# Luh1124/face-vae

Hardware: AMD Instinct MI355X
Metric: training images/sec (256x256 face-VAE step) (higher is better)
Workload: dtype bf16; 1 GPU; FaceVAE step 256x256 (AFE trunk + reparam + Generator trunk, MSE+KL, Adam); global_batch=32, per_gpu_batch=32, resolution=256, parallelism=dp1

## Files before the change

### face-vae_amd/csrc/conv.hip

```cpp
#include "conv_plan.h"

namespace {

__global__ void weight_prep_c7n_kernel(const float* __restrict__ wp, const float* sigma, bf16* wn, int cout) {
  const float inv = sigma ? 1.f / sigma[0] : 1.f;
  for (int e = blockIdx.x * blockDim.x + threadIdx.x; e < 32 * 448; e += gridDim.x * blockDim.x) {
    const int nn = e / 448, k = e - nn * 448;
    const int co = nn / 7, s = nn - co * 7, r = k >> 6, ci = k & 63;
    const float v = co < cout ? wp[((co * 64 + ci) * 7 + r) * 7 + s] * inv : 0.f;
    wn[e] = (bf16)v;
  }
}

template <typename T>
__device__ __forceinline__ void weight_prep_body(const float* __restrict__ wp, const float* sigma, T* wk, int rows,
                                                 int Kpad, int cout, int cin_valid, int lgCin, int KS, int K,
                                                 int transposed, int bid, int nblk, int smaj = 0) {
  const int total = rows * Kpad;
  const float inv = sigma ? 1.f / sigma[0] : 1.f;
  for (int e = bid * (int)blockDim.x + threadIdx.x; e < total; e += nblk * (int)blockDim.x) {
    int row, k;
    bool kin;
    int tap, c;
    if (smaj == 2) {
// ... 716 lines not shown
  const int dtype = descs[0].dtype;
  for (int i = 0; i < n; ++i) {
    const fv_conv_desc* d = &descs[i];
    int st = check_desc(d);
    if (st) return st;
    FV_REQUIRE(d->dtype == dtype, "weight_prep_multi: one dtype per call");
    FV_REQUIRE(fv_conv_weight_prep_batchable(d), "weight_prep_multi: conv %d needs a special layout", i);
    FV_REQUIRE(w_params[i] && wks[i], "weight_prep_multi: null pointer (conv %d)", i);
    const int ks = d->ksize;
    WPrepMJob j0{w_params[i], sigmas[i], wks[i], wrows(d->cout), kpad_lay(smaj_wk(d), kpad_of(ks, d->cin)),
                 fv_ilog2(d->cin),
                 ks * ks * d->cin, 0, 0, d->cout, d->cin_valid, ks, 0, smaj_wk(d)};
    j0.nb = (int)std::min<long>(fv_cdiv((long)j0.rows * j0.Kpad, 256), 256);
    nb_total = std::max(nb_total, j0.nb);
    m.j[m.n++] = j0;
    if (wts[i]) {
      const int cin_t = pad_pow2_8(d->cout);
      WPrepMJob j1{w_params[i], sigmas[i], wts[i], wrows(d->cin), kpad_lay(smaj_wt(d), kpad_of(ks, cin_t)),
                   fv_ilog2(cin_t),
                   ks * ks * cin_t, 1, 0, d->cout, d->cin_valid, ks, 0, smaj_wt(d)};
      j1.nb = (int)std::min<long>(fv_cdiv((long)j1.rows * j1.Kpad, 256), 256);
      nb_total = std::max(nb_total, j1.nb);
      m.j[m.n++] = j1;
    }
  }
  hipStream_t s = (hipStream_t)stream;
  if (dtype == FV_BF16)
    hipLaunchKernelGGL(weight_prep_multi_kernel<bf16>, dim3(nb_total, m.n), dim3(256), 0, s, m);
  else
    hipLaunchKernelGGL(weight_prep_multi_kernel<float>, dim3(nb_total, m.n), dim3(256), 0, s, m);
  return fv_check_launch("weight_prep_multi");
}

static int sr_geometry(const fv_conv_desc* d, int* bp) {
  if (d->dtype != FV_BF16 || use_c7n(d) || halo_tr(d) || use_subpix(d) || use_c64(d)) return 0;
  const int bn = halo3_bn(d);
  const long P = (long)d->n * d->h * d->w;
  if (!bn || d->cout % bn || P % 256) return 0;
  const int nw = bn == 64 ? 4 : 8;
  if (bp) *bp = 256 / nw;
  return (int)(P / 256 * nw);
}

extern "C++" {
static int cu_count() {
  static int n = 0;
  if (!n) {
    int dev = 0;
    if (hipGetDevice(&dev) != hipSuccess || hipDeviceGetAttribute(&n, hipDeviceAttributeMultiprocessorCount, dev) != hipSuccess ||
        n <= 0)
      n = 256;
  }
  return n;
}
static bool halo_epi_ok(const ConvArgs& a, int bn, int tr) {
  return a.lgtw == 6 && !a.sub && !a.nchw && a.W % 64 == 0 && a.H % tr == 0 && a.P == a.N * a.H * a.W &&
         a.ntn * bn == a.Cout && a.ldy >= a.Cout;
}
static int launch_h3(int bn, int mode, int ntiles, hipStream_t s, const ConvArgs& a, unsigned xb) {
  const int sch = res_sched(2) >= 2 ? 2 : 0;
  const char* e = getenv("FV_PERS_GRID");
  const int cap = (e && atoi(e) > 0) ? atoi(e) : cu_count();
  const bool pers = bn < 256 && ntiles > cap;
  if (!launch_halo3_fwd3(a, bn, mode, sch, pers, pers ? cap : ntiles, xb, ntiles, s)) return FV_OK;
  fv_set_error("halo 3x3 conv variant unsupported (co tile %d, mode %d)", bn, mode);
  return FV_E_BADARG;
}
static int launch_h2(int bn, int nblk, hipStream_t s, const ConvArgs& a, unsigned xb) {
  if (!launch_halo3_fwd2(a, bn, nblk, xb, s)) return FV_OK;
  fv_set_error("halo 3x3 conv variant unsupported (co tile %d)", bn);
  return FV_E_BADARG;
}
}

static bool use_c1s(const fv_conv_desc* d) {
  const char* e = getenv("FV_C1S");
  if (e && e[0] == '0') return false;
  if (!use_v2(d) || d->ksize != 1 || d->upsample || d->pro_act) return false;
  if ((d->cin != 256 && d->cin != 512) || d->cout % 256 || d->ldy != d->cout) return false;
  const long P = (long)d->n * d->h * d->w;
  return P % (32768 / d->cin) == 0 && P * d->cout * 2 < (1L << 31);
}

static int conv_run(const fv_conv_desc* d, const void* x, const void* wk, const float* bias,
                    const float* psc, const float* psh, const void* res, void* y, float* stats,
                    hipStream_t s, const fv_store_reduce* sr = nullptr) {
  ConvArgs a{};
  if (sr && sr->mode) {
    FV_REQUIRE(sr_geometry(d, nullptr) > 0, "store-pass records not available for this conv (query fv_conv2d_sr_records)");
    FV_REQUIRE(sr->records, "store-pass records: null buffer");
    FV_REQUIRE(sr->mode == 1 || (sr->mode == 2 && sr->bn_input && sr->mean && sr->invstd && sr->gamma && sr->beta && !res),
               "store-pass records: bad mode / BN arguments");
    FV_REQUIRE(!stats, "store-pass records and accumulator statistics in one call are not supported");
    a.spm = sr->mode;
    a.sprec = sr->records;
    a.bnm = sr->mean; a.bni = sr->invstd; a.bng = sr->gamma; a.bnb = sr->beta; a.bns = sr->slope;
    if (sr->mode == 2) res = sr->bn_input;
  }
  const FwdTile t = fwd_tile(d->cout);
  a.x = x; a.w = wk; a.bias = bias; a.psc = psc; a.psh = psh; a.slope = d->pro_slope;
  a.res = res; a.y = y; a.stats = stats;
  a.nrec = stats ? fv_conv2d_stats_blocks(d) : 0;
  a.N = d->n; a.H = d->h; a.W = d->w;
  a.Hin = d->upsample ? d->h / 2 : d->h;
  a.Win = d->upsample ? d->w / 2 : d->w;
  a.P = d->n * d->h * d->w;
  a.Cin = d->cin; a.lgCin = fv_ilog2(d->cin);
  a.Cout = d->cout; a.ldy = d->ldy;
  a.K = d->ksize * d->ksize * d->cin; a.Kpad = kpad_of(d->ksize, d->cin); a.nks = a.Kpad / BK;
  a.sigmoid = d->epi_sigmoid; a.nchw = d->out_nchw_f32;
  a.ntn = fv_cdiv(d->cout, t.bn);
  int st;
  const long wk_have = (long)fv_conv_wk_elems(d);
  auto wext = [&](long rows, long kk, const char* what) {
    if (rows * kk > wk_have) {
      fv_set_error("conv %s: weight DMA extent %ld x %ld > weight image %ld elements", what, rows, kk, wk_have);
      return FV_E_BADARG;
    }
    return FV_OK;
  };
  if (use_c7n(d)) {
    FV_REQUIRE(!res, "out_conv kernel: no residual");
    const unsigned xb = (unsigned)((long)d->n * d->h * d->w * 64 * 2);
    const int band = c7n_band(d);
    const int nblk = d->n * (d->h / band) * (d->w / 64);
    launch_c7n(a, nblk, xb, band, s);
    return fv_check_launch("conv2d_fwd_c7n2");
  }
  const bool c64 = use_c64(d);
  if (c64 && !res && !a.spm) {
    if ((st = wext(d->cout, kpad_of(3, 64), "c64"))) return st;
    const int nb = c64_bands(d);
    const int nblk = d->n * (d->w / 64) * (d->cout / 64) * nb;
    const unsigned xb = (unsigned)((long)d->n * d->h * d->w * 64 * 2);
    launch_c64(a, nblk, xb, nb, s);
    return fv_check_launch("conv2d_fwd_c64");
  }
  if (use_c74(d)) {
    FV_REQUIRE(!res, "packed 7x7 conv: no residual");
    const int ntiles = d->n * (d->h / C74_TR) * (d->w / 64);
    const unsigned xb = (unsigned)((long)d->n * d->h * d->w * d->cin * 2);
    FV_REQUIRE(!a.stats || a.nrec == c74_grid(d), "packed 7x7 conv: %d BN records for %d blocks", a.nrec, c74_grid(d));
    launch_c74(a, c74_grid(d), xb, ntiles, s);
    return fv_check_launch("conv2d_fwd_c74");
  }
  if (const int tr = halo_tr(d)) {
    if ((st = wext(plan_tile(d).bn, kpad_of(7, d->cin), "halo7"))) return st;
    a.lgtw = 6;
    const int nblk = d->n * (d->h / tr) * (d->w / 64);
    const unsigned xb = (unsigned)((long)d->n * d->h * d->w * d->cin * 2);
    if (launch_halo7(a, d->cin, nblk, xb, s)) {
      fv_set_error("7x7 halo conv variant unsupported (cin=%d)", d->cin);
      return FV_E_BADARG;
    }
    return fv_check_launch("conv2d_fwd_halo");
  }
  if (use_upband(d)) {
    FV_REQUIRE(!res && !a.spm, "sub-pixel band conv: no residual / store-pass records");
    a.Ho = d->h; a.Wo = d->w;
    a.Kpad = kpad_of(2, d->cin);
    a.wphase = wrows(d->cout) * a.Kpad;
    if ((st = wext(4L * wrows(d->cout), a.Kpad, "upband"))) return st;
    const int hl = d->h / 2, wl = d->w / 2;
    const long base = (long)d->n * (wl / 32) * (d->cout / 64);
    int nb = 1;
    while (base * nb < 256 && hl % (nb * 16) == 0) nb *= 2;
    const int nblk = (int)(base * nb);
    const unsigned xb = (unsigned)((long)d->n * hl * wl * 128 * 2);
    launch_upband(a, nblk, xb, nb, s);
    return fv_check_launch("conv2d_fwd_upband");
  }
  if (use_subpix_halo(d)) {
// ... 97 lines not shown
  return fv_check_launch("conv2d_fwd");
}

int fv_conv2d_fwd(const fv_conv_desc* d, const void* x, const void* wk, const float* bias,
                  const float* pro_scale, const float* pro_shift, const void* res, void* y,
                  float* stats, void* stream) {
  int st = check_desc(d);
  if (st) return st;
  FV_REQUIRE(x && wk && y, "null pointer");
  FV_REQUIRE(!d->pro_act || (pro_scale && pro_shift), "prologue needs scale/shift");
  FV_REQUIRE(d->out_nchw_f32 || d->ldy >= d->cout, "ldy < cout");
  FV_REQUIRE(!res || d->ldy % 4 == 0, "residual needs ldy % 4 == 0");
  FV_REQUIRE(d->out_nchw_f32 || d->cout % 4 == 0 || d->ldy >= d->cout, "bad ldy");
  return conv_run(d, x, wk, bias, pro_scale, pro_shift, res, y, stats, (hipStream_t)stream);
}

static fv_conv_desc dgrad_desc(const fv_conv_desc* d) {
  fv_conv_desc t{};
  t.dtype = d->dtype;
  t.n = d->n; t.h = d->h; t.w = d->w;
  t.cin = pad_pow2_8(d->cout);
  t.cin_valid = d->cout;
  t.cout = d->cin;
  t.ldy = d->cin;
  t.ksize = d->ksize;
  return t;
}

int fv_conv2d_sr_records(const fv_conv_desc* d, int dgrad, int* record_pixels) {
  if (check_desc(d) != FV_OK) return 0;
  if (dgrad) {
    if (d->upsample) return 0;
    const fv_conv_desc t = dgrad_desc(d);
    return sr_geometry(&t, record_pixels);
  }
  return sr_geometry(d, record_pixels);
}

int fv_conv2d_fwd_sr(const fv_conv_desc* d, const void* x, const void* wk, const float* bias, const void* res, void* y,
                     const fv_store_reduce* sr, void* stream) {
  int st = check_desc(d);
  if (st) return st;
  FV_REQUIRE(x && wk && y && sr && sr->mode == 1, "fwd_sr: null pointer or mode != 1");
  FV_REQUIRE(!d->pro_act && !d->out_nchw_f32 && d->ldy == d->cout, "fwd_sr: plain NHWC output only");
  return conv_run(d, x, wk, bias, nullptr, nullptr, res, y, nullptr, (hipStream_t)stream, sr);
}

int fv_conv2d_bwd_data_sr(const fv_conv_desc* d, const void* dy, int ldy_dy, const void* wt, void* dx,
                          const fv_store_reduce* sr, void* stream) {
  int st = check_desc(d);
  if (st) return st;
  FV_REQUIRE(dy && wt && dx && sr && sr->mode == 2 && !d->upsample, "bwd_data_sr: bad argument");
  const fv_conv_desc t = dgrad_desc(d);
  FV_REQUIRE(ldy_dy == t.cin, "bwd_data: dy channel stride must be %d (got %d)", t.cin, ldy_dy);
  return conv_run(&t, dy, wt, nullptr, nullptr, nullptr, nullptr, dx, nullptr, (hipStream_t)stream, sr);
}

int fv_conv2d_bwd_data(const fv_conv_desc* d, const void* dy, int ldy_dy, const void* wt, void* dx,
                       void* stream) {
  int st = check_desc(d);
  if (st) return st;
  const fv_conv_desc t = dgrad_desc(d);
  FV_REQUIRE(ldy_dy == t.cin, "bwd_data: dy channel stride must be %d (got %d)", t.cin, ldy_dy);
  if (const int bn = dgrad_halo_bn(d)) {
    FV_REQUIRE(dy && wt && dx, "null pointer");
    ConvArgs a{};
    a.x = dy; a.w = wt; a.y = dx;
// ... 1450 lines not shown
```

### face-vae_amd/csrc/conv_shapes.hip

```cpp
#include "conv_plan.h"

namespace {

template <int KS, int CIN, int RN, int TR, bool WLDS, bool KSPLIT>
__global__ void __launch_bounds__(512, 4)
conv_halo_fwd(ConvArgs a, unsigned x_bytes) {
  constexpr int PAD = KS / 2, TW = 64;
  constexpr int MT = TR * 4;
  constexpr int RM = KSPLIT ? MT : MT / 8;
  constexpr int HR = TR + KS - 1, HW = TW + KS - 1;
  constexpr int CPP = CIN / 8;
  constexpr int HCH = HR * HW * CPP;
  constexpr int HQ = (HCH + 63) / 64;
  constexpr int KPAD = ((KS * KS * CIN + 31) / 32) * 32;
  constexpr int NKS = KPAD / 32;
  constexpr int KPW = (NKS + 7) / 8;
  constexpr int WROW = KPAD / 8 + 1;
  constexpr int WCH = RN * 16 * WROW;
  constexpr int WQ = WLDS ? (WCH + 63) / 64 : 0;
  constexpr int HB = HQ * 1024, WB = WQ * 1024;
  constexpr int SCR = 4096;
  static_assert(!KSPLIT || (RN == 1 && !WLDS && 8 * MT * 1024 <= HB), "k-split layout");
  __shared__ __attribute__((aligned(1024))) char smem[HB + WB + SCR];
  char* halo = smem;
// ... 85 lines not shown
#pragma unroll 2
    for (int ks = ks0; ks < ks1; ++ks) {
      const int kc = ks * 4 + g;
      bf16x8 bfr[RN];
#pragma unroll
      for (int nn = 0; nn < RN; ++nn) {
        if constexpr (WLDS) bfr[nn] = *reinterpret_cast<const bf16x8*>(wlds + ((nn * 16 + li) * WROW + kc) * 16);
        else bfr[nn] = *reinterpret_cast<const bf16x8*>(wk + (long)(nn * 16 + li) * a.Kpad + kc * 8);
      }
      kstep(ks, bfr);
    }
  }
  const int p0 = (n * a.H + h0) * a.W + w0;
  if constexpr (KSPLIT) {
    __syncthreads();
    f32x4* red = reinterpret_cast<f32x4*>(halo);
#pragma unroll
    for (int m = 0; m < RM; ++m) red[(wave * RM + m) * 64 + lane] = acc[0][m];
    __syncthreads();
    f32x4 t[1][1];
    t[0][0] = f32x4{0.f, 0.f, 0.f, 0.f};
#pragma unroll
    for (int w = 0; w < 8; ++w) t[0][0] += red[(w * RM + wave) * 64 + lane];
    conv_epilogue<bf16, 1, 8, 1, 1>(a, t, smem + HB + WB, 0, p0, tile, 0, wave, lane, tid);
  } else {
    conv_epilogue<bf16, 1, 8, RN, RM>(a, acc, smem + HB + WB, 0, p0, tile, 0, wave, lane, tid);
  }
}

constexpr int C74_HW = 71, C74_HR = C74_TR + 6;
constexpr int C74_WCOL = C74_K / 8;
constexpr int C74_WQ = 64 * C74_WCOL / 64;
constexpr int C74_HQ = (C74_HR * C74_HW + 63) / 64;
__global__ void __launch_bounds__(512, 2)
conv7c4_fwd(ConvArgs a, unsigned x_bytes, int ntiles) {
  constexpr int WB = C74_WQ * 1024, HB = C74_HQ * 1024, NHB = 3;
  __shared__ __attribute__((aligned(1024))) char smem[WB + NHB * HB];
  const int tid = threadIdx.x, lane = tid & 63;
  const int wave = __builtin_amdgcn_readfirstlane(tid >> 6);
  const int li = lane & 15, g = lane >> 4;
  const int tiles_w = a.W >> 6, tiles_h = a.H / C74_TR;
  const unsigned sbase = __builtin_amdgcn_readfirstlane((unsigned)(size_t)(lds_ptr_t)smem);
  const __amdgpu_buffer_rsrc_t xr = __builtin_amdgcn_make_buffer_rsrc(const_cast<void*>(a.x), 0, (int)x_bytes, 0x00020000);
  const __amdgpu_buffer_rsrc_t wr = __builtin_amdgcn_make_buffer_rsrc(const_cast<void*>(a.w), 0, 0x7fffffff, 0x00020000);

  auto issue_halo = [&](int tile, int buf) {
    const int n = tile / (tiles_h * tiles_w), rem = tile - n * tiles_h * tiles_w;
    const int h0 = (rem / tiles_w) * C74_TR, w0 = (rem % tiles_w) * 64;
    for (int q = wave; q < C74_HQ; q += 8) {
      const int L = q * 64 + lane;
      const int hr = L / C74_HW, hc = L - (L / C74_HW) * C74_HW;
      const int hh = h0 + hr - 3, ww = w0 + hc - 3;
      const bool ok = L < C74_HR * C74_HW && hh >= 0 && hh < a.H && ww >= 0 && ww < a.W;
      dma16s(xr, sbase + WB + buf * HB + q * 1024, ok ? (unsigned)((((n * a.H + hh) * a.W + ww) * 8) * 2) : 0x80000000u, 0u);
    }
  };
  for (int q = wave; q < C74_WQ; q += 8) {
    const int L = q * 64 + lane;
    const int li = L & 15, t = L >> 4, col = t % C74_WCOL, row = (t / C74_WCOL) * 16 + li;
    dma16s(wr, sbase + q * 1024, (unsigned)((row * C74_K + col * 8) * 2), 0u);
  }
  int tile = blockIdx.x;
  if (tile < ntiles) issue_halo(tile, 0);
  if (tile + (int)gridDim.x < ntiles) issue_halo(tile + gridDim.x, 1);
  asm volatile("s_waitcnt vmcnt(0)" ::: "memory");
  __syncthreads();

  float bv[4][4];
#pragma unroll
  for (int nn = 0; nn < 4; ++nn)
#pragma unroll
    for (int i = 0; i < 4; ++i) bv[nn][i] = a.bias ? a.bias[nn * 16 + g * 4 + i] : 0.f;
  int hbase[2];
#pragma unroll
  for (int m = 0; m < 2; ++m) {
    const int loc = wave * 32 + m * 16 + li;
    hbase[m] = (loc >> 6) * C74_HW + (loc & 63);
  }
  float bs[4][4], bq[4][4];
#pragma unroll
  for (int nn = 0; nn < 4; ++nn)
#pragma unroll
    for (int i = 0; i < 4; ++i) bs[nn][i] = bq[nn][i] = 0.f;
  int buf = 0;
  for (; tile < ntiles; tile += gridDim.x) {
    const int ahead = tile + 2 * gridDim.x;
    if (ahead < ntiles) issue_halo(ahead, buf == 0 ? 2 : buf - 1);
    f32x4 acc[4][2];
#pragma unroll
    for (int nn = 0; nn < 4; ++nn)
#pragma unroll
      for (int m = 0; m < 2; ++m) acc[nn][m] = f32x4{0.f, 0.f, 0.f, 0.f};
    const char* hs = smem + WB + buf * HB;
#pragma unroll
    for (int r = 0; r < 7; ++r) {
      bf16x8 bfr[4], afr[2];
#pragma unroll
      for (int nn = 0; nn < 4; ++nn)
        bfr[nn] = *reinterpret_cast<const bf16x8*>(smem + ((nn * C74_WCOL + r * 4 + g) * 16 + li) * 16);
#pragma unroll
      for (int m = 0; m < 2; ++m) {
        const char* p = hs + (hbase[m] + r * C74_HW + 2 * g) * 16;
        const uint2 lo = *reinterpret_cast<const uint2*>(p), hi = *reinterpret_cast<const uint2*>(p + 16);
        afr[m] = __builtin_bit_cast(bf16x8, make_uint4(lo.x, lo.y, hi.x, hi.y));
      }
#pragma unroll
      for (int nn = 0; nn < 4; ++nn)
#pragma unroll
        for (int m = 0; m < 2; ++m) acc[nn][m] = __builtin_amdgcn_mfma_f32_16x16x32_bf16(bfr[nn], afr[m], acc[nn][m], 0, 0, 0);
    }
    const int n = tile / (tiles_h * tiles_w), rem = tile - n * tiles_h * tiles_w;
    const int p0 = (n * a.H + (rem / tiles_w) * C74_TR) * a.W + (rem % tiles_w) * 64;
#pragma unroll
    for (int nn = 0; nn < 4; ++nn)
#pragma unroll
      for (int m = 0; m < 2; ++m)
#pragma unroll
        for (int i = 0; i < 4; ++i) acc[nn][m][i] += bv[nn][i];
    if (a.stats) {
#pragma unroll
      for (int nn = 0; nn < 4; ++nn)
#pragma unroll
        for (int i = 0; i < 4; ++i) {
          const float v0 = acc[nn][0][i], v1 = acc[nn][1][i];
          bs[nn][i] += v0 + v1;
          bq[nn][i] += v0 * v0 + v1 * v1;
        }
    }
    auto pk = [](float lo, float hi) {
      const bf16 t[2] = {(bf16)lo, (bf16)hi};
      return *reinterpret_cast<const unsigned*>(t);
    };
#pragma unroll
    for (int m = 0; m < 2; ++m) {
      const int loc = wave * 32 + m * 16 + li;
      bf16* yp = reinterpret_cast<bf16*>(a.y) + (long)(p0 + (loc >> 6) * a.W + (loc & 63)) * a.ldy;
#pragma unroll
      for (int q = 0; q < 2; ++q) {
        const f32x4 va = acc[2 * q][m], vb = acc[2 * q + 1][m];
        const auto s0 = __builtin_amdgcn_permlane16_swap(pk(va[0], va[1]), pk(vb[0], vb[1]), false, false);
        const auto s1 = __builtin_amdgcn_permlane16_swap(pk(va[2], va[3]), pk(vb[2], vb[3]), false, false);
        *reinterpret_cast<uint4*>(yp + (2 * q + (g & 1)) * 16 + (g >> 1) * 8) = make_uint4(s0[0], s1[0], s0[1], s1[1]);
      }
    }
    {
      const int dpieces = ahead < ntiles ? (wave + 8 < C74_HQ ? 2 : 1) : 0;
      wait_vm_dyn(8 + dpieces);
    }
    wait_lgkm0();
    __builtin_amdgcn_s_barrier();
    asm volatile("" ::: "memory");
    buf = buf == 2 ? 0 : buf + 1;
  }
  if (a.stats) {
    float* sw = reinterpret_cast<float*>(smem + WB);
#pragma unroll
    for (int nn = 0; nn < 4; ++nn)
#pragma unroll
      for (int i = 0; i < 4; ++i) {
        const float sv = row16_sum(bs[nn][i]), qv = row16_sum(bq[nn][i]);
        if (li == 0) {
          sw[wave * 128 + nn * 16 + g * 4 + i] = sv;
          sw[wave * 128 + 64 + nn * 16 + g * 4 + i] = qv;
        }
      }
    __syncthreads();
    if (tid < 128 && (int)blockIdx.x < a.nrec) {
      float v = 0.f;
#pragma unroll
      for (int w = 0; w < 8; ++w) v += sw[w * 128 + tid];
      a.stats[(long)blockIdx.x * 128 + tid] = v;
    }
  }
}

constexpr int C64_PXB = 160, C64_ROWB = 11 * 1024, C64_NR = 10;
__global__ void __launch_bounds__(512, 1)
conv3c64_fwd(ConvArgs a, unsigned x_bytes, int nbands) {
  __shared__ __attribute__((aligned(1024))) char smem[C64_NR * C64_ROWB];
  __shared__ __attribute__((aligned(16))) float sbias[64];
  __shared__ __attribute__((aligned(16))) float sacc[8 * 16 * 64];
  const int tid = threadIdx.x, lane = tid & 63;
  const int wave = __builtin_amdgcn_readfirstlane(tid >> 6);
  const int cg = wave & 1, rw = wave >> 1;
  const int lr = lane & 15, lh = lane >> 4;
// ... 504 lines not shown
    const int h0 = hb + 4 * j;
    for (int o = tid; o < nout; o += 512) {
      const int co = o / (C7_TR * 64), rr = (o / 64) % C7_TR, w = o % 64;
      float v = co == 0 ? bias4[0] : co == 1 ? bias4[1] : co == 2 ? bias4[2] : bias4[3];
#pragma unroll
      for (int s7 = 0; s7 < 7; ++s7) v += Dl[(rr * 70 + w + s7) * C7B_DLD + co * 7 + s7];
      if (a.stats) {
        const float sv = wave_sum(v), qv = wave_sum(v * v);
        const int rec = ((n * a.H + h0 + rr) * a.W + w0) >> 6;
        if (lane == 0 && rec < a.nrec) {
          a.stats[(long)(rec * 2) * a.Cout + co] = sv;
          a.stats[(long)(rec * 2 + 1) * a.Cout + co] = qv;
        }
      }
      if (a.sigmoid) v = 1.f / (1.f + expf(-v));
      const int pix = (h0 + rr) * a.W + w0 + w;
      if (a.nchw) reinterpret_cast<float*>(a.y)[((long)(n * a.Cout + co)) * HWo + pix] = v;
      else reinterpret_cast<bf16*>(a.y)[((long)n * HWo + pix) * a.ldy + co] = (bf16)v;
    }
  }
}


}

int launch_halo7(const ConvArgs& a, int cin, int nblk, unsigned xb, hipStream_t s) {
  if (cin == 8) hipLaunchKernelGGL((conv_halo_fwd<7, 8, 4, 4, true, false>), dim3(nblk), dim3(512), 0, s, a, xb);
  else if (cin == 64) hipLaunchKernelGGL((conv_halo_fwd<7, 64, 1, 2, false, true>), dim3(nblk), dim3(512), 0, s, a, xb);
  else return FV_E_UNSUPPORTED;
  return FV_OK;
}

void launch_c74(const ConvArgs& a, int grid, unsigned xb, int ntiles, hipStream_t s) {
  hipLaunchKernelGGL(conv7c4_fwd, dim3(grid), dim3(512), 0, s, a, xb, ntiles);
}

void launch_c64(const ConvArgs& a, int nblk, unsigned xb, int nbands, hipStream_t s) {
  hipLaunchKernelGGL(conv3c64_fwd, dim3(nblk), dim3(512), 0, s, a, xb, nbands);
}

void launch_upband(const ConvArgs& a, int nblk, unsigned xb, int nbands, hipStream_t s) {
  hipLaunchKernelGGL(conv3up_band_fwd, dim3(nblk), dim3(512), 0, s, a, xb, nbands);
}

int launch_c1s(const ConvArgs& a, int k, int bpx, int grid, unsigned xb, hipStream_t s) {
  if (k == 256 && bpx == 128) hipLaunchKernelGGL((conv1x1_stream<256, 128>), dim3(grid), dim3(512), 0, s, a, xb);
  else if (k == 256 && bpx == 64) hipLaunchKernelGGL((conv1x1_stream<256, 64>), dim3(grid), dim3(512), 0, s, a, xb);
  else if (k == 512 && bpx == 64) hipLaunchKernelGGL((conv1x1_stream<512, 64>), dim3(grid), dim3(512), 0, s, a, xb);
  else if (k == 512 && bpx == 32) hipLaunchKernelGGL((conv1x1_stream<512, 32>), dim3(grid), dim3(512), 0, s, a, xb);
  else return FV_E_UNSUPPORTED;
  return FV_OK;
}

void launch_c7n(const ConvArgs& a, int nblk, unsigned xb, int band, hipStream_t s) {
  hipLaunchKernelGGL(conv7_n3_fwd2, dim3(nblk), dim3(512), 0, s, a, xb, band);
}
```

### face-vae_amd/ops.py

```python
from __future__ import annotations

import ctypes
import os
import weakref
from typing import Optional

import torch

from . import _lib as L
from ._lib import call, ptr, query, stream

CL = torch.channels_last
F32 = torch.float32
F64 = torch.float64
FP8 = torch.float8_e4m3fn
_FP8_HANDOFF = True


def storage(mode: torch.dtype) -> torch.dtype:
    return torch.bfloat16 if mode == FP8 else mode


def fp8_site(conv, which: str, device):
    sites = conv.__dict__.setdefault("_fv_fp8_sites", {})
    st = sites.get(which)
    if st is None or st[0].device != device:
        st = [torch.zeros(query("fv_fp8_site_bytes") // 4, dtype=torch.int32, device=device), False, []]
        sites[which] = st
    return st


FP8_GLOBAL = None


def _dq_snapshot(site):
    if site is None or len(site) < 3:
        return
    for ref in site[2]:
        cs = ref()
        q = getattr(cs, "x8", None) if cs is not None else None
        if q is not None and q[1].data_ptr() == site[0].data_ptr() + 18 * 4:
            cs.x8 = (q[0], q[1].clone())
    site[2].clear()


_DQ_VIEW = os.environ.get("FV_DQ_VIEW", "1") == "1"


def _hold_x8(cs, x8, xdq, site):
# ... 308 lines not shown
    if stats:
        nb, _ = stats_geometry(cs)
        part = _empty(nb * 2 * d.cout, F32, x.device)
    psc, psh = (pro if pro is not None else (None, None))
    if cs.fp8:
        site = fp8_site(cs.conv, "x", x.device)
        x8, xdq = x8 if x8 is not None else quantize_fp8_site(x, site)
        _hold_x8(cs, x8, xdq, site)
        _timed("fwd", d, lambda: call("fv_conv2d_fwd_fp8_site", ctypes.byref(d), ptr(x8), ptr(site[0]), ptr(cs.wk),
                                      ptr(cs.wdq), ptr(bias), ptr(res), ptr(y), ptr(part), stream()))
        if CHECK is not None:
            CHECK("fwd", cs, x=x, bias=bias, pro=pro, res=res, y=y, q8=(x8, xdq))
        return part
    _timed("fwd", d, lambda: call("fv_conv2d_fwd", ctypes.byref(d), ptr(x), ptr(cs.wk), ptr(bias), ptr(psc),
                                  ptr(psh), ptr(res), ptr(y), ptr(part), stream()))
    if CHECK is not None:
        CHECK("fwd", cs, x=x, bias=bias, pro=pro, res=res, y=y)
    return part


def sr_records(d, dgrad):
    bp = ctypes.c_int(0)
    nrec = query("fv_conv2d_sr_records", ctypes.byref(d), int(dgrad), ctypes.byref(bp))
    return (nrec, bp.value) if nrec > 0 else None


class BNRecords:
    __slots__ = ("part", "nb", "bp", "dx")

    def __init__(self, part, nb, bp, dx):
        self.part, self.nb, self.bp, self.dx = part, nb, bp, dx


def _dgrad_bnred(cs, dy, dx, bnred):
    d = cs.d
    if bnred is None or cs.fp8 or d.upsample or d.dtype != L.FV_BF16:
        return None
    geo = sr_records(d, True)
    if geo is None:
        return None
    bn, r, ybn, slope = bnred
    if r.count == 0 and r.stats is None:
        return None
    nb, bp = geo
    part = _empty(nb * 2 * d.cin, F32, dy.device)
    sr = L.StoreReduce(2, ptr(part), ptr(ybn), ptr(r.mean), ptr(r.invstd), ptr(bn.weight), ptr(bn.bias),
                       float(slope))
    _timed("dgrad", d, lambda: call("fv_conv2d_bwd_data_sr", ctypes.byref(d), ptr(dy), d.cout, ptr(cs.wt), ptr(dx),
                                    ctypes.byref(sr), stream()))
    return BNRecords(part, nb, bp, dx)


def _wgrad(cs: ConvState, x, dy, ldd, pro, need_db):
    d = cs.d
    dev = dy.device
    slab = _empty(query("fv_conv2d_wgrad_slab_elems", ctypes.byref(d)), F32, dev)
    bslab = _empty(query("fv_conv2d_wgrad_bias_slab_elems", ctypes.byref(d)), F32, dev) if need_db else None
    psc, psh = (pro if pro is not None else (None, None))
    _timed("wgrad", d, lambda: call("fv_conv2d_bwd_weight", ctypes.byref(d), ptr(x), ptr(psc), ptr(psh), ptr(dy),
                                    ldd, ptr(slab), ptr(bslab), stream()))
    return _wgrad_finish(cs, x, dy, ldd, pro, need_db, slab, bslab)


def _wgrad_fp8(cs: ConvState, x, dy, ldd, need_db, dy8):
    d = cs.d
    dev = dy.device
    x8, xdq = cs.x8
    dy8_, dydq = dy8
    slab = _empty(query("fv_conv2d_wgrad_slab_elems", ctypes.byref(d)), F32, dev)
    bslab = _empty(query("fv_conv2d_wgrad_bias_slab_elems", ctypes.byref(d)), F32, dev) if need_db else None
    _timed("wgrad", d, lambda: call("fv_conv2d_bwd_weight_fp8", ctypes.byref(d), ptr(x8), ptr(xdq), ptr(dy8_), ptr(dydq),
                                    ptr(slab), ptr(bslab), stream()))
    cs.x8 = None
    return _wgrad_finish(cs, x, dy, ldd, None, need_db, slab, bslab, q8=(x8, xdq, dy8_, dydq))


def _wgrad_finish(cs: ConvState, x, dy, ldd, pro, need_db, slab, bslab, q8=None):
    d = cs.d
    dev = dy.device
    dw = torch.empty_like(cs.w)
    db = torch.empty(d.cout, dtype=F32, device=dev) if need_db else None
# ... 61 lines not shown
        site = fp8_site(cs.conv, "dy", dy.device)
        dy8 = dy8 if dy8 is not None else quantize_fp8_site(dy, site)
        dw, db = _wgrad_fp8(cs, x, dy, ldd, need_db, dy8)
    else:
        if x.numel() == 0 or (dy.numel() == 0 and dy8 is None):
            raise RuntimeError("conv backward: the bf16 operand of this fp8 conv was never materialised "
                               "(FV_Q8_ONLY) and its e4m3 copy was released by an earlier backward; "
                               "backward through an fp8 ResBlock runs once (no retain_graph)")
        dw, db = _wgrad(cs, x, dy, ldd, pro, need_db)
    dx, recs = _dgrad(cs, dy, ldd, need_dx, bnred, dy8)
    return (dx, dw, db, recs) if want_recs else (dx, dw, db)


def _dgrad(cs: ConvState, dy, ldd, need_dx, bnred, dy8=None):
    d = cs.d
    dev = dy.device
    if not need_dx:
        return None, None
    if cs.fp8:
        site = fp8_site(cs.conv, "dy", dy.device)
        dy8, dydq = dy8 if dy8 is not None else quantize_fp8_site(dy, site)
        dx = torch.empty((d.n, d.cin, d.h, d.w), dtype=dy.dtype, device=dev, memory_format=CL)
        _timed("dgrad", d, lambda: call("fv_conv2d_bwd_data_fp8_site", ctypes.byref(d), ptr(dy8), ptr(site[0]),
                                        ptr(cs.wt), ptr(cs.wdq), ptr(dx), stream()))
        if CHECK is not None:
            CHECK("dgrad", cs, dy=dy, ldd=ldd, dx=dx, q8=(dy8, dydq))
        return dx, None
    if d.upsample and query("fv_conv2d_dgrad_lowres", ctypes.byref(d)):
        dx = torch.empty((d.n, d.cin, d.h // 2, d.w // 2), dtype=dy.dtype, device=dev, memory_format=CL)
        _timed("dgrad", d, lambda: call("fv_conv2d_bwd_data", ctypes.byref(d), ptr(dy), ldd, ptr(cs.wt), ptr(dx),
                                        stream()))
    else:
        dx = torch.empty((d.n, d.cin, d.h, d.w), dtype=dy.dtype, device=dev, memory_format=CL)
        recs = _dgrad_bnred(cs, dy, dx, bnred) if ldd == d.cout else None
        if recs is not None:
            if CHECK is not None:
                CHECK("dgrad", cs, dy=dy, ldd=ldd, dx=dx)
            return dx, recs
        _timed("dgrad", d, lambda: call("fv_conv2d_bwd_data", ctypes.byref(d), ptr(dy), ldd, ptr(cs.wt), ptr(dx),
                                        stream()))
        if d.upsample:
            src = torch.empty((d.n, d.cin, d.h // 2, d.w // 2), dtype=dy.dtype, device=dev, memory_format=CL)
            call("fv_upsample2x_bwd", L.dtype_code(dy.dtype), ptr(dx), d.n, d.h // 2, d.w // 2, d.cin, ptr(src),
                 stream())
            dx = src
    if CHECK is not None:
        CHECK("dgrad", cs, dy=dy, ldd=ldd, dx=dx)
    return dx, None



class BNResult:
    __slots__ = ("mean", "invstd", "scale", "shift", "count", "stats")


def _bn_result(C, dev, count, stats=None):
    r = BNResult()
    r.mean = torch.empty(C, dtype=F32, device=dev)
    r.invstd = torch.empty(C, dtype=F32, device=dev)
    r.scale = torch.empty(C, dtype=F32, device=dev)
    r.shift = torch.empty(C, dtype=F32, device=dev)
    r.count = count
    r.stats = stats
    return r


def _running(bn, training):
# ... 339 lines not shown
        ctx.blk, ctx.cs, ctx.r, ctx.comm = blk, cs, r, comm
        ctx.save_for_backward(x, xb, a)
        return y

    @staticmethod
    def backward(ctx, dy):
        x, xb, a = ctx.saved_tensors
        blk, cs, r = ctx.blk, ctx.cs, ctx.r
        dy = grad_in(dy, xb.dtype)
        da, dw, db = conv_backward(cs, a, dy, dy.shape[1])
        dxb, dg, dbt = bn_act_backward(da, xb, blk.bn, r, blk.slope, False, ctx.comm,
                                       need_dx=ctx.needs_input_grad[0])
        return (from_nhwc(dxb, x) if dxb is not None else None), dw, db, dg, dbt, None


class ConvFn(torch.autograd.Function):

    @staticmethod
    def forward(ctx, x, weight, bias, conv, mode, sigmoid):
        dtype = storage(mode)
        xb, cin_pad = to_nhwc(x, dtype)
        N, _, H, W = x.shape
        cout = conv.out_channels
        nchw = bool(sigmoid) or (cout % 8 != 0)
        d = desc(dtype, N, H, W, cin_pad, conv.in_channels, cout, cout, conv.kernel_size, sig=sigmoid, nchw=nchw)
        cs = ConvState(conv, d, dtype, x.device, conv.training, need_wt=ctx.needs_input_grad[0], fp8=mode == FP8)
        if nchw:
            y = torch.empty((N, cout, H, W), dtype=F32, device=x.device)
        else:
            y = torch.empty((N, cout, H, W), dtype=dtype, device=x.device, memory_format=CL)
        conv_forward(cs, xb, bias, y=y)
        cs.release()
        ctx.cs, ctx.sigmoid, ctx.nchw, ctx.dtype = cs, sigmoid, nchw, dtype
        ctx.save_for_backward(x, xb, y if sigmoid else None)
        return y

    @staticmethod
    def backward(ctx, dy):
        x, xb, y = ctx.saved_tensors
        cs = ctx.cs
        d = cs.d
        dtype = ctx.dtype
        if ctx.nchw:
            ldd = pad_pow2(d.cout)
            dpre = torch.empty((d.n, ldd, d.h, d.w), dtype=dtype, device=dy.device, memory_format=CL)
            dy32 = dy.float().contiguous()
            if ctx.sigmoid:
                call("fv_sigmoid_bwd_to_nhwc", L.dtype_code(dtype), ptr(dy32), ptr(y), d.n, d.cout, d.h * d.w, ldd,
                     ptr(dpre), stream())
            else:
                call("fv_nchw_to_nhwc", L.dtype_code(dtype), ptr(dy32), d.n, d.cout, d.h * d.w, ldd, ptr(dpre),
                     stream())
        else:
            ldd = d.cout
            dpre = grad_in(dy, dtype)
        dxb, dw, db = conv_backward(cs, xb, dpre, ldd, need_dx=ctx.needs_input_grad[0])
        dx = from_nhwc(dxb, x) if dxb is not None else None
        return dx, dw, db, None, None, None



class S2ConvState:

    def __init__(self, conv, d, in_hw, dtype, device, training, need_wt):
        self.conv, self.d, self.in_hw = conv, d, in_hw
        w = conv.weight_param()
        if w.dtype != F32 or not w.is_contiguous():
            raise RuntimeError("conv weights must be contiguous fp32")
        self.w = w
        self.sigma = None
        self.fp8 = False
        if conv.sn:
            pre = getattr(conv, "_sn_pre", None)
            if pre is not None:
                self.sigma, self.u, self.v = pre
                conv._sn_pre = None
            else:
                self.sigma = spectral_norm_fwd(w, conv.weight_u, conv.weight_v, training)
                self.u = conv.weight_u.clone()
                self.v = conv.weight_v.clone()
        conv._fv_desc = conv._fv_prep = conv._fv_desc8 = conv._fv_prep8 = None
        self.wk = _empty(query("fv_conv2d_s2_wk_elems", ctypes.byref(d)), dtype, device)
        self.wt = _empty(query("fv_conv2d_s2_wt_elems", ctypes.byref(d)), dtype, device) if need_wt else None
        call("fv_conv2d_s2_weight_prep", ctypes.byref(d), ptr(w), ptr(self.sigma), ptr(self.wk), ptr(self.wt), stream())

    def release(self):
        self.wk = None


# ... 371 lines not shown
```

Measured before the change: 2847 images/s.

## Fuse BN/LeakyReLU backward reduction into packed 7x7 dgrad conv store pass

```diff
diff --git a/face-vae_amd/csrc/conv.hip b/face-vae_amd/csrc/conv.hip
--- a/face-vae_amd/csrc/conv.hip
+++ b/face-vae_amd/csrc/conv.hip
@@ -772,7 +772,13 @@
   return fv_check_launch("weight_prep_multi");
 }
 
-static int sr_geometry(const fv_conv_desc* d, int* bp) {
+static int sr_geometry(const fv_conv_desc* d, int* bp, int mode = 1) {
+  if (mode == 2 && d->dtype == FV_BF16 && use_c74(d)) {
+    const int ntiles = d->n * (d->h / C74_TR) * (d->w / 64), tpb = c74_tiles_per_block(d);
+    if (ntiles % tpb) return 0;
+    if (bp) *bp = tpb * C74_TR * 64;
+    return c74_grid(d);
+  }
   if (d->dtype != FV_BF16 || use_c7n(d) || halo_tr(d) || use_subpix(d) || use_c64(d)) return 0;
   const int bn = halo3_bn(d);
   const long P = (long)d->n * d->h * d->w;
@@ -827,7 +833,7 @@
                     hipStream_t s, const fv_store_reduce* sr = nullptr) {
   ConvArgs a{};
   if (sr && sr->mode) {
-    FV_REQUIRE(sr_geometry(d, nullptr) > 0, "store-pass records not available for this conv (query fv_conv2d_sr_records)");
+    FV_REQUIRE(sr_geometry(d, nullptr, sr->mode) > 0, "store-pass records not available for this conv (query fv_conv2d_sr_records)");
     FV_REQUIRE(sr->records, "store-pass records: null buffer");
     FV_REQUIRE(sr->mode == 1 || (sr->mode == 2 && sr->bn_input && sr->mean && sr->invstd && sr->gamma && sr->beta && !res),
                "store-pass records: bad mode / BN arguments");
@@ -877,7 +883,7 @@
     return fv_check_launch("conv2d_fwd_c64");
   }
   if (use_c74(d)) {
-    FV_REQUIRE(!res, "packed 7x7 conv: no residual");
+    FV_REQUIRE(a.spm == 2 ? !bias : (!res && !a.spm), "packed 7x7 conv: no residual / mode-1 records; no bias with mode 2");
     const int ntiles = d->n * (d->h / C74_TR) * (d->w / 64);
     const unsigned xb = (unsigned)((long)d->n * d->h * d->w * d->cin * 2);
     FV_REQUIRE(!a.stats || a.nrec == c74_grid(d), "packed 7x7 conv: %d BN records for %d blocks", a.nrec, c74_grid(d));
@@ -1041,7 +1047,7 @@
   if (dgrad) {
     if (d->upsample) return 0;
     const fv_conv_desc t = dgrad_desc(d);
-    return sr_geometry(&t, record_pixels);
+    return sr_geometry(&t, record_pixels, 2);
   }
   return sr_geometry(d, record_pixels);
 }
diff --git a/face-vae_amd/csrc/conv_shapes.hip b/face-vae_amd/csrc/conv_shapes.hip
--- a/face-vae_amd/csrc/conv_shapes.hip
+++ b/face-vae_amd/csrc/conv_shapes.hip
@@ -141,10 +141,12 @@
 constexpr int C74_WCOL = C74_K / 8;
 constexpr int C74_WQ = 64 * C74_WCOL / 64;
 constexpr int C74_HQ = (C74_HR * C74_HW + 63) / 64;
-__global__ void __launch_bounds__(512, 2)
+template <int REC>
+__global__ void __launch_bounds__(512, REC == 2 ? 4 : 2)
 conv7c4_fwd(ConvArgs a, unsigned x_bytes, int ntiles) {
   constexpr int WB = C74_WQ * 1024, HB = C74_HQ * 1024, NHB = 3;
-  __shared__ __attribute__((aligned(1024))) char smem[WB + NHB * HB];
+  constexpr int PB = WB + NHB * HB;
+  __shared__ __attribute__((aligned(1024))) char smem[PB + (REC == 2 ? 1024 : 0)];
   const int tid = threadIdx.x, lane = tid & 63;
   const int wave = __builtin_amdgcn_readfirstlane(tid >> 6);
   const int li = lane & 15, g = lane >> 4;
@@ -156,8 +158,10 @@
   auto issue_halo = [&](int tile, int buf) {
     const int n = tile / (tiles_h * tiles_w), rem = tile - n * tiles_h * tiles_w;
     const int h0 = (rem / tiles_w) * C74_TR, w0 = (rem % tiles_w) * 64;
+    int hlane = lane;
+    if constexpr (REC == 2) asm volatile("" : "+v"(hlane));
     for (int q = wave; q < C74_HQ; q += 8) {
-      const int L = q * 64 + lane;
+      const int L = q * 64 + hlane;
       const int hr = L / C74_HW, hc = L - (L / C74_HW) * C74_HW;
       const int hh = h0 + hr - 3, ww = w0 + hc - 3;
       const bool ok = L < C74_HR * C74_HW && hh >= 0 && hh < a.H && ww >= 0 && ww < a.W;
@@ -172,6 +176,30 @@
   int tile = blockIdx.x;
   if (tile < ntiles) issue_halo(tile, 0);
   if (tile + (int)gridDim.x < ntiles) issue_halo(tile + gridDim.x, 1);
+  uint4 ybn[REC == 2 ? 4 : 1];
+  auto chunk_ofs = [&]() -> unsigned {
+    int ol = lane;
+    asm volatile("" : "+v"(ol));
+    const int oi = ol & 15, og = ol >> 4;
+    return (unsigned)((((wave >> 1) * a.W + (wave & 1) * 32 + oi) * 64 + (og & 1) * 16 + (og >> 1) * 8) * 2);
+  };
+  auto tile_bytes = [&](int t) -> long {
+    const int n = t / (tiles_h * tiles_w), rem = t - n * tiles_h * tiles_w;
+    return (long)((n * a.H + (rem / tiles_w) * C74_TR) * a.W + (rem % tiles_w) * 64) * 128;
+  };
+  auto load_ybn = [&](int t) {
+    const char* ub = reinterpret_cast<const char*>(a.res) + tile_bytes(t);
+    const unsigned cofs = chunk_ofs();
+#pragma unroll
+    for (int c = 0; c < 4; ++c) ybn[c] = *reinterpret_cast<const uint4*>(ub + cofs + (c >> 1) * 2048 + (c & 1) * 64);
+  };
+  if constexpr (REC == 2) {
+    if (tid < 256) {
+      const float* src = tid < 64 ? a.bnm : tid < 128 ? a.bni : tid < 192 ? a.bng : a.bnb;
+      reinterpret_cast<float*>(smem + PB)[tid] = src[tid & 63];
+    }
+    if (tile < ntiles) load_ybn(tile);
+  }
   asm volatile("s_waitcnt vmcnt(0)" ::: "memory");
   __syncthreads();
 
@@ -179,7 +207,7 @@
 #pragma unroll
   for (int nn = 0; nn < 4; ++nn)
 #pragma unroll
-    for (int i = 0; i < 4; ++i) bv[nn][i] = a.bias ? a.bias[nn * 16 + g * 4 + i] : 0.f;
+    for (int i = 0; i < 4; ++i) bv[nn][i] = (REC == 0 && a.bias) ? a.bias[nn * 16 + g * 4 + i] : 0.f;
   int hbase[2];
 #pragma unroll
   for (int m = 0; m < 2; ++m) {
@@ -191,10 +219,15 @@
   for (int nn = 0; nn < 4; ++nn)
 #pragma unroll
     for (int i = 0; i < 4; ++i) bs[nn][i] = bq[nn][i] = 0.f;
+  f32x2 gs[2][4], gq[2][4];
+#pragma unroll
+  for (int q = 0; q < 2; ++q)
+#pragma unroll
+    for (int k = 0; k < 4; ++k) gs[q][k] = gq[q][k] = f32x2{0.f, 0.f};
   int buf = 0;
   for (; tile < ntiles; tile += gridDim.x) {
     const int ahead = tile + 2 * gridDim.x;
-    if (ahead < ntiles) issue_halo(ahead, buf == 0 ? 2 : buf - 1);
+    if (REC == 0 && ahead < ntiles) issue_halo(ahead, buf == 0 ? 2 : buf - 1);
     f32x4 acc[4][2];
 #pragma unroll
     for (int nn = 0; nn < 4; ++nn)
@@ -220,13 +253,15 @@
     }
     const int n = tile / (tiles_h * tiles_w), rem = tile - n * tiles_h * tiles_w;
     const int p0 = (n * a.H + (rem / tiles_w) * C74_TR) * a.W + (rem % tiles_w) * 64;
-#pragma unroll
-    for (int nn = 0; nn < 4; ++nn)
-#pragma unroll
-      for (int m = 0; m < 2; ++m)
-#pragma unroll
-        for (int i = 0; i < 4; ++i) acc[nn][m][i] += bv[nn][i];
-    if (a.stats) {
+    if constexpr (REC == 0) {
+#pragma unroll
+      for (int nn = 0; nn < 4; ++nn)
+#pragma unroll
+        for (int m = 0; m < 2; ++m)
+#pragma unroll
+          for (int i = 0; i < 4; ++i) acc[nn][m][i] += bv[nn][i];
+    }
+    if (REC == 0 && a.stats) {
 #pragma unroll
       for (int nn = 0; nn < 4; ++nn)
 #pragma unroll
@@ -240,6 +275,8 @@
       const bf16 t[2] = {(bf16)lo, (bf16)hi};
       return *reinterpret_cast<const unsigned*>(t);
     };
+    unsigned cofs = 0;
+    if constexpr (REC == 2) cofs = chunk_ofs();
 #pragma unroll
     for (int m = 0; m < 2; ++m) {
       const int loc = wave * 32 + m * 16 + li;
@@ -249,17 +286,67 @@
         const f32x4 va = acc[2 * q][m], vb = acc[2 * q + 1][m];
         const auto s0 = __builtin_amdgcn_permlane16_swap(pk(va[0], va[1]), pk(vb[0], vb[1]), false, false);
         const auto s1 = __builtin_amdgcn_permlane16_swap(pk(va[2], va[3]), pk(vb[2], vb[3]), false, false);
-        *reinterpret_cast<uint4*>(yp + (2 * q + (g & 1)) * 16 + (g >> 1) * 8) = make_uint4(s0[0], s1[0], s0[1], s1[1]);
-      }
+        const uint4 out = make_uint4(s0[0], s1[0], s0[1], s1[1]);
+        if constexpr (REC == 0) *reinterpret_cast<uint4*>(yp + (2 * q + (g & 1)) * 16 + (g >> 1) * 8) = out;
+        else *reinterpret_cast<uint4*>(reinterpret_cast<char*>(a.y) + tile_bytes(tile) + cofs + m * 2048 + q * 64) = out;
+        if constexpr (REC == 2) {
+          const int c = (2 * q + (g & 1)) * 16 + (g >> 1) * 8;
+          const float* bp = reinterpret_cast<const float*>(smem + PB) + c;
+          Chunk8<bf16> v, r;
+          v.raw = out;
+          r.raw = ybn[m * 2 + q];
+#pragma unroll
+          for (int k = 0; k < 4; ++k) {
+            const f32x2 bm_ = *reinterpret_cast<const f32x2*>(bp + 2 * k), bi_ = *reinterpret_cast<const f32x2*>(bp + 64 + 2 * k);
+            const f32x2 bg_ = *reinterpret_cast<const f32x2*>(bp + 128 + 2 * k), bb_ = *reinterpret_cast<const f32x2*>(bp + 192 + 2 * k);
+            const f32x2 rr = {r.get(2 * k), r.get(2 * k + 1)}, gv = {v.get(2 * k), v.get(2 * k + 1)};
+            const f32x2 yh = (rr - bm_) * bi_;
+            const f32x2 t = bg_ * yh + bb_;
+            const f32x2 sl = gv * a.bns;
+            const f32x2 gg = {t.x > 0.f ? gv.x : sl.x, t.y > 0.f ? gv.y : sl.y};
+            gs[q][k] += gg;
+            gq[q][k] = f32x2{__builtin_fmaf(gg.x, yh.x, gq[q][k].x), __builtin_fmaf(gg.y, yh.y, gq[q][k].y)};
+          }
+#pragma unroll
+          for (int k = 0; k < 4; ++k) asm volatile("" : "+v"(gs[q][k]), "+v"(gq[q][k]));
+          __builtin_amdgcn_sched_barrier(0);
+        }
+      }
+    }
+    if constexpr (REC == 2) {
+      if (ahead < ntiles) issue_halo(ahead, buf == 0 ? 2 : buf - 1);
+      if (tile + (int)gridDim.x < ntiles) load_ybn(tile + gridDim.x);
     }
     {
       const int dpieces = ahead < ntiles ? (wave + 8 < C74_HQ ? 2 : 1) : 0;
-      wait_vm_dyn(8 + dpieces);
+      wait_vm_dyn(REC == 2 ? 12 + dpieces : 8 + dpieces);
     }
     wait_lgkm0();
     __builtin_amdgcn_s_barrier();
     asm volatile("" ::: "memory");
     buf = buf == 2 ? 0 : buf + 1;
+  }
+  if constexpr (REC == 2) {
+    float* sw = reinterpret_cast<float*>(smem + WB);
+#pragma unroll
+    for (int q = 0; q < 2; ++q)
+#pragma unroll
+      for (int j = 0; j < 8; ++j) {
+        const float sv = row16_sum(gs[q][j >> 1][j & 1]), qv = row16_sum(gq[q][j >> 1][j & 1]);
+        if (li == 0) {
+          const int c = (2 * q + (g & 1)) * 16 + (g >> 1) * 8 + j;
+          sw[wave * 128 + c] = sv;
+          sw[wave * 128 + 64 + c] = qv;
+        }
+      }
+    __syncthreads();
+    if (tid < 128) {
+      float v = 0.f;
+#pragma unroll
+      for (int w = 0; w < 8; ++w) v += sw[w * 128 + tid];
+      a.sprec[(long)blockIdx.x * 128 + tid] = v;
+    }
+    return;
   }
   if (a.stats) {
     float* sw = reinterpret_cast<float*>(smem + WB);
@@ -830,7 +917,8 @@
 }
 
 void launch_c74(const ConvArgs& a, int grid, unsigned xb, int ntiles, hipStream_t s) {
-  hipLaunchKernelGGL(conv7c4_fwd, dim3(grid), dim3(512), 0, s, a, xb, ntiles);
+  if (a.spm == 2) hipLaunchKernelGGL(conv7c4_fwd<2>, dim3(grid), dim3(512), 0, s, a, xb, ntiles);
+  else hipLaunchKernelGGL(conv7c4_fwd<0>, dim3(grid), dim3(512), 0, s, a, xb, ntiles);
 }
 
 void launch_c64(const ConvArgs& a, int nblk, unsigned xb, int nbands, hipStream_t s) {
diff --git a/face-vae_amd/ops.py b/face-vae_amd/ops.py
--- a/face-vae_amd/ops.py
+++ b/face-vae_amd/ops.py
@@ -15,6 +15,7 @@
 F64 = torch.float64
 FP8 = torch.float8_e4m3fn
 _FP8_HANDOFF = True
+BNRED_FUSED = True
 
 
 def storage(mode: torch.dtype) -> torch.dtype:
@@ -389,9 +390,9 @@
         self.part, self.nb, self.bp, self.dx = part, nb, bp, dx
 
 
-def _dgrad_bnred(cs, dy, dx, bnred):
+def _dgrad_bnred(cs, dy, ldd, dx, bnred):
     d = cs.d
-    if bnred is None or cs.fp8 or d.upsample or d.dtype != L.FV_BF16:
+    if not BNRED_FUSED or bnred is None or cs.fp8 or d.upsample or d.dtype != L.FV_BF16:
         return None
     geo = sr_records(d, True)
     if geo is None:
@@ -403,7 +404,7 @@
     part = _empty(nb * 2 * d.cin, F32, dy.device)
     sr = L.StoreReduce(2, ptr(part), ptr(ybn), ptr(r.mean), ptr(r.invstd), ptr(bn.weight), ptr(bn.bias),
                        float(slope))
-    _timed("dgrad", d, lambda: call("fv_conv2d_bwd_data_sr", ctypes.byref(d), ptr(dy), d.cout, ptr(cs.wt), ptr(dx),
+    _timed("dgrad", d, lambda: call("fv_conv2d_bwd_data_sr", ctypes.byref(d), ptr(dy), ldd, ptr(cs.wt), ptr(dx),
                                     ctypes.byref(sr), stream()))
     return BNRecords(part, nb, bp, dx)
 
@@ -531,7 +532,7 @@
                                         stream()))
     else:
         dx = torch.empty((d.n, d.cin, d.h, d.w), dtype=dy.dtype, device=dev, memory_format=CL)
-        recs = _dgrad_bnred(cs, dy, dx, bnred) if ldd == d.cout else None
+        recs = _dgrad_bnred(cs, dy, ldd, dx, bnred)
         if recs is not None:
             if CHECK is not None:
                 CHECK("dgrad", cs, dy=dy, ldd=ldd, dx=dx)
@@ -937,6 +938,7 @@
         conv_forward(cs, xb, bias, y=y)
         cs.release()
         ctx.cs, ctx.sigmoid, ctx.nchw, ctx.dtype = cs, sigmoid, nchw, dtype
+        ctx.src = _claim_bnsrc(x, xb)
         ctx.save_for_backward(x, xb, y if sigmoid else None)
         return y
 
@@ -959,7 +961,10 @@
         else:
             ldd = d.cout
             dpre = grad_in(dy, dtype)
-        dxb, dw, db = conv_backward(cs, xb, dpre, ldd, need_dx=ctx.needs_input_grad[0])
+        dxb, dw, db, recs_in = conv_backward(cs, xb, dpre, ldd, need_dx=ctx.needs_input_grad[0],
+                                             bnred=_bnred_of(ctx.src), want_recs=True)
+        if ctx.src is not None:
+            ctx.src["recs"] = recs_in
         dx = from_nhwc(dxb, x) if dxb is not None else None
         return dx, dw, db, None, None, None
 
```

Measured after the change: 2859 images/s (median of 6 runs). No clear change (+0.4%).
